# N-HANS/N-HANS

Measured on AMD Instinct MI355X. Metric: denoised audio seconds per second (16 kHz), whole job, higher is better.
Workload: dtype f16x3 (split hi+lo f16 operands, f32 accumulate); 1 GPU; 256 x 10 s 16 kHz synthetic mixture(s) per GPU, denoiser model, STFT+embed+mask+iSTFT end-to-end; clips_per_gpu=256, distinct_clips_per_gpu=256, frames_per_gpu=255488, weights=synthetic seed 7, parallelism=clip-sharded x1

## Files before the change

### include/nhans_hip.h

```cpp
#ifndef NHANS_HIP_H
#define NHANS_HIP_H

#include <stddef.h>
#include <stdint.h>

#ifdef __cplusplus
extern "C" {
#endif

#define NHANS_ABI_VERSION 5

#define NHANS_DENOISER 0
#define NHANS_SEPARATOR 1

#define NHANS_OK 0
#define NHANS_EINVAL (-1)
#define NHANS_EHIP (-2)
#define NHANS_ENOMEM (-3)
#define NHANS_ESHORT (-4)

#define NHANS_STATUS_SATURATED 1

#define NHANS_NUM_ACTIVATIONS 25

// ... 31 lines not shown

int nhans_embed(nhans_ctx* ctx, const float* ctx_logmag_dev, int n, float* emb_out_dev, void* stream);

int nhans_mask_net(nhans_ctx* ctx, const float* logmag_dev, const int64_t* frame_offsets_host,
                   int nclips, const float* emb_a_dev, const float* emb_b_dev,
                   float* logits_out_dev, float* denoised_out_dev, void* stream);

int nhans_istft(nhans_ctx* ctx, const float* logmag_dev, const float* phase_dev,
                const int64_t* frame_offsets_host, int nclips, const int64_t* out_offsets_host,
                float* wav_out_dev, void* stream);

int nhans_enhance_clips(nhans_ctx* ctx, const float* mix_wav_dev, const int64_t* mix_offsets_host,
                        int nclips, const float* ctx_a_wav_dev, const int64_t* ctx_a_offsets_host,
                        const float* ctx_b_wav_dev, const int64_t* ctx_b_offsets_host,
                        float* denoised_wav_dev, float* mixed_wav_dev, float* logmag_out_dev,
                        float* phase_out_dev, float* logits_out_dev, float* emb_out_dev, void* stream);

int nhans_debug_block_output(nhans_ctx* ctx, const float* logmag_dev, const int64_t* frame_offsets_host,
                             int nclips, const float* emb_a_dev, const float* emb_b_dev,
                             int64_t frame0, int nframes, int block, float* out_dev, void* stream);

int nhans_debug_activation(nhans_ctx* ctx, const float* logmag_dev, const int64_t* frame_offsets_host,
                           int nclips, const float* emb_a_dev, const float* emb_b_dev,
                           int64_t frame0, int nframes, int index, float* out_dev, void* stream);
int nhans_debug_tower_activation(nhans_ctx* ctx, const float* ctx_logmag_dev, int n, int index, float* out_dev,
                                 void* stream);

int nhans_take_status(nhans_ctx* ctx, int* flags_out, void* stream);

int nhans_debug_launch_probe(size_t dynamic_lds_bytes, void* stream);

int nhans_debug_mfma_ceiling(double seconds, void* stream, double* sustained_tflops, double* first_tflops,
                             int* launches);

uint32_t nhans_crc32c(uint32_t crc, const void* data_host, size_t nbytes);

typedef struct nhans_online nhans_online;

int nhans_online_open(nhans_ctx* ctx, int nstreams, const float* ctx_a_wav_dev, const int64_t* ctx_a_offsets_host,
                      const float* ctx_b_wav_dev, const int64_t* ctx_b_offsets_host, int want_mixed, void* stream,
                      nhans_online** out);

int nhans_online_open_slots(nhans_ctx* ctx, int nslots, int want_mixed, void* stream, nhans_online** out);

int nhans_online_restart(nhans_online* obj, int slot);

int nhans_online_set_context(nhans_online* obj, int slot, const float* ctx_a_wav_dev, int64_t na,
                             const float* ctx_b_wav_dev, int64_t nb, void* stream, int64_t* first_frame_out);

int nhans_online_set_embeddings(nhans_online* obj, int slot, const float* emb_a_dev, const float* emb_b_dev,
                                void* stream, int64_t* first_frame_out);


int nhans_online_push(nhans_online* obj, const float* in_dev, const int64_t* in_offsets_host, const int* end_host,
                      float* den_out_dev, float* mixed_out_dev, const int64_t* out_offsets_host,
                      int64_t* out_counts_host, void* stream);

int nhans_online_out_counts(const nhans_online* obj, const int64_t* in_counts_host, const int* end_host,
                            int64_t* out_counts_host);

int nhans_online_rewind(nhans_online* obj);

int nhans_online_set_lookahead(nhans_online* obj, int slot, int lookahead);

void nhans_online_close(nhans_online* obj);

// ... 96 lines not shown
```

### n-hans_amd/csrc/conv_epilogue.h

```cpp
#pragma once
#include "nhans_kernels.h"
#include <cstddef>

namespace nhans {

typedef float f32x16 __attribute__((ext_vector_type(16)));
typedef float f32x4 __attribute__((ext_vector_type(4)));
typedef _Float16 f16x8 __attribute__((ext_vector_type(8)));
typedef _Float16 f16x4 __attribute__((ext_vector_type(4)));

template <int I, int NM, int ND> __device__ __forceinline__ void pin_reads_between_mfmas() {
    if constexpr (I < ND) {
        __builtin_amdgcn_sched_group_barrier(0x008, (I + 1) * NM / ND - I * NM / ND, 0);
        __builtin_amdgcn_sched_group_barrier(0x100, 1, 0);
        pin_reads_between_mfmas<I + 1, NM, ND>();
    }
}

template <int I, int NM, int ND> __device__ __forceinline__ void pin_reads_front_loaded() {
    if constexpr (I < ND) {
        __builtin_amdgcn_sched_group_barrier(0x008, 1, 0);
        __builtin_amdgcn_sched_group_barrier(0x100, 1, 0);
        pin_reads_front_loaded<I + 1, NM, ND>();
    } else if constexpr (NM > ND) {
// ... 253 lines not shown
    int* const satp = CONV_KARG(sat);
    if (sat && satp) atomicOr(satp, kSatActivation);
}

template <int TM, int TN, int PREC, int NTHREADS, int BMROWS, int BNCOLS>
__device__ __forceinline__ void conv_epilogue(const ConvArgs& a, f32x16 (&acc)[TM][TN], float* smem, EpiTile tile,
                                              int row_base, int col_base, int n_tile0, int tid, int lane,
                                              long long* es = nullptr ) {
    constexpr int LDC = BNCOLS + 4;
    constexpr int C4 = BNCOLS / 4;
    constexpr int PP = NTHREADS / C4;
    constexpr int PASSES = BMROWS / PP;
    float* ct = smem;
    int4* rowinfo = reinterpret_cast<int4*>(smem + BMROWS * LDC);

#pragma unroll
    for (int i = 0; i < TM; ++i)
#pragma unroll
        for (int j = 0; j < TN; ++j)
#pragma unroll
            for (int g = 0; g < 4; ++g) {
                const f32x4 v = {acc[i][j][4 * g], acc[i][j][4 * g + 1], acc[i][j][4 * g + 2], acc[i][j][4 * g + 3]};
                *reinterpret_cast<f32x4*>(ct + (row_base + i * 32 + (lane & 31)) * LDC + col_base + j * 32 + 8 * g +
                                          4 * (lane >> 5)) = v;
            }
    if (tid < BMROWS) {
        const int mz = tile(tid, a);
        const int m = mz < 0 ? (tile.tw > 0 ? tile(0, a) : a.M - 1) : mz;
        const uint32_t b = fd_div((uint32_t)m, a.fdHoWo);
        const uint32_t rem = (uint32_t)m - b * a.fdHoWo.d;
        const uint32_t ho = fd_div(rem, a.fdWo);
        const uint32_t wo = rem - ho * a.fdWo.d;
        const int clip = a.img_clip ? a.img_clip[b] : 0;
        int ids;
        if (a.id_mode == 2 && a.id_win.t) {
            const int h = (int)ho * a.idsh;
            ids = win_row_ok(a.id_win, (int)b, h) ? win_row(a.id_win, (int)b, h) * a.idW + (int)wo * a.idsw : kNoRow;
        } else {
            ids = (int)((b * a.idH + ho * a.idsh) * a.idW + wo * a.idsw);
        }
        rowinfo[tid] = make_int4(clip * a.cb_stride, (int)rem * a.N, mz, ids);
    }
    if (kDev && es) { asm volatile("s_waitcnt lgkmcnt(0)" ::: "memory"); es[0] = (long long)__builtin_amdgcn_s_memtime(); }
    __syncthreads();
    if (kDev && es) es[1] = (long long)__builtin_amdgcn_s_memtime();

    const int c4 = tid % C4, prow = tid / C4;
    const int n = n_tile0 + c4 * 4;
    const int f_tf = a.tf ? 1 : 0;
    const bool id_split = a.id_mode == 1 && a.id_split;
    const float* __restrict__ cbp = a.cb;
    const float* __restrict__ tfp = a.tf ? a.tf : a.zero;
    const bool vec = (a.Nreal == a.N) && !a.aux && (a.out_split || (a.ldo & 3) == 0) &&
                     (a.id_mode != 1 || id_split || (a.id_ld & 3) == 0);
    constexpr int C8 = BNCOLS / 8, PP8 = NTHREADS / C8, PASSES8 = BMROWS / PP8;
    if (vec && a.epi8 && a.out_split && (a.id_mode == 0 || id_split || a.id_mode == 2)) {
        const int c8 = tid % C8, prow8 = tid / C8;
        const int n8 = n_tile0 + c8 * 8;
        const bool one_clip = rowinfo[0].x == rowinfo[BMROWS - 1].x;
        const int mode8 = (a.id_mode == 0 ? 0 : a.id_mode == 1 ? 1 : 2) * 2 + (one_clip ? 1 : 0);
        switch (mode8) {
            case 0: conv_epilogue_sweep8<PREC, 0, 0, PP8, PASSES8, LDC>(a, ct, rowinfo, prow8, c8, n8, es); break;
            case 1: conv_epilogue_sweep8<PREC, 0, 1, PP8, PASSES8, LDC>(a, ct, rowinfo, prow8, c8, n8, es); break;
            case 2: conv_epilogue_sweep8<PREC, 1, 0, PP8, PASSES8, LDC>(a, ct, rowinfo, prow8, c8, n8, es); break;
            case 3: conv_epilogue_sweep8<PREC, 1, 1, PP8, PASSES8, LDC>(a, ct, rowinfo, prow8, c8, n8, es); break;
            case 4: conv_epilogue_sweep8<PREC, 3, 0, PP8, PASSES8, LDC>(a, ct, rowinfo, prow8, c8, n8, es); break;
            default: conv_epilogue_sweep8<PREC, 3, 1, PP8, PASSES8, LDC>(a, ct, rowinfo, prow8, c8, n8, es); break;
        }
    } else if (vec) {
        const int mode = (a.id_mode == 1 ? (id_split ? 1 : 2) : a.id_mode == 2 ? 3 : 0) * 2 + (a.out_split ? 1 : 0);
        switch (mode) {
            case 0: conv_epilogue_sweep<PREC, 0, 0, PP, PASSES, LDC>(a, ct, rowinfo, prow, c4, n); break;
            case 1: conv_epilogue_sweep<PREC, 0, 1, PP, PASSES, LDC>(a, ct, rowinfo, prow, c4, n); break;
            case 2: conv_epilogue_sweep<PREC, 1, 0, PP, PASSES, LDC>(a, ct, rowinfo, prow, c4, n); break;
// ... 35 lines not shown
```

### n-hans_amd/csrc/conv_igemm_halo.hip

```cpp
#include "conv_epilogue.h"
#include <cstdlib>

namespace nhans {

namespace {
constexpr int NCW = 8;
constexpr int NPW = 4;

template <int HBM_> struct HaloShape {
    static constexpr int HBM = HBM_;
    static constexpr int HR = HBM_ == 512 ? 544 : 320;
    static constexpr int BST = HBM_ == 512 ? 3 : 4;
    static constexpr int WN = HBM_ == 512 ? 1 : 2;
    static constexpr int NAP = HR * 8 / (NPW * 64);
};

template <int N> __device__ __forceinline__ void halo_wait_vmcnt() {
    asm volatile("s_waitcnt vmcnt(%0)" ::"n"(N) : "memory");
}
}

template <int BN, int PREC, int HBM_ = 256, int DBG = 0, int ABL = 0, int PWM = 0>
__global__ void __launch_bounds__((NCW + NPW) * 64) conv_igemm_halo(const ConvArgs a) {
    using SH = HaloShape<HBM_>;
// ... 106 lines not shown
                                     (__attribute__((address_space(3))) void*)(DST), 16, 0, 0);

        int segA = 0, khA = 0, ccA = 0, supA = 0, kwA = 0;
#define NH_ISSUE_A(BUF)                                                                            \
    {                                                                                              \
        const int khoff_ = (khA * sW + (PWM ? kwA : 0)) * sC + ccA * 32;                           \
        const bool live_ = supA < nsup;                                                            \
        float* sa_ = smem + (BUF) * A_BUF + pw * 8 * 32;                                           \
        _Pragma("unroll") for (int d = 0; d < NAPW; ++d) {                                         \
            bool in_ = !(ABL & 1) && live_ && (unsigned)(hov[d] + khA) < (unsigned)sH;             \
            if constexpr (PWM) in_ = in_ && (unsigned)(wiv[d] + kwA) < (unsigned)sW;               \
            if constexpr (!(ABL & 2))                                                              \
                __builtin_amdgcn_raw_ptr_buffer_load_lds(srsrc, (__attribute__((address_space(3))) void*)(sa_ + d * 32 * 32), 16, \
                                                         in_ ? (unsigned)(poff[d] + khoff_ * 4) : kOob, 0, 0, 0); \
        }                                                                                          \
        ++supA;                                                                                    \
        if (PWM && ++kwA < KW0) {                  \
        } else if (kwA = 0, ++khA >= (segA ? KH1 : KH0)) {  \
            khA = 0;                                                                               \
            if (++ccA >= (segA ? CC1 : CC0)) {                                                     \
                ccA = 0;                                                                           \
                if (segA == 0 && nseg > 1) {                                                       \
                    segA = 1;                                                                      \
                    NH_MAP_SEGMENT(1)                                                              \
                }                                                                                  \
            }                                                                                      \
        }                                                                                          \
    }
        int tapB = 0;
        const __amdgpu_buffer_rsrc_t wr0 = __builtin_amdgcn_make_buffer_rsrc(const_cast<float*>(a.seg[0].wpk) + (size_t)nt0 * 1024, 0, 0x7FFFFFFF, 0x00020000);
        const __amdgpu_buffer_rsrc_t wr1 = __builtin_amdgcn_make_buffer_rsrc(const_cast<float*>(nseg > 1 ? a.seg[1].wpk : a.seg[0].wpk) + (size_t)nt0 * 1024, 0, 0x7FFFFFFF, 0x00020000);
        const unsigned wvo = (unsigned)ptid * 16u;
        const int bstride_b = (int)(bstride * 4);
        int wtap = -1, wseg = 0;
#define NH_ISSUE_B(ST)                                                                             \
    {                                                                                              \
        if (tapB < total && !(ABL & 4)) {                                                          \
            if (tapB == ntap0) { wseg = 1; wtap = 0; } else ++wtap;                                \
        }                                                                                          \
        ++tapB;                                                                                    \
        float* sb_ = smem + B_BASE + (ST) * B_STAGE;                                               \
        const int so_ = (ABL & 4) ? 0 : wtap * bstride_b;                                          \
        _Pragma("unroll") for (int j = 0; j < GBP; ++j)                                            \
            if constexpr (!(ABL & 8))                                                              \
                __builtin_amdgcn_raw_ptr_buffer_load_lds((wseg || (ABL & 4)) ? wr1 : wr0,          \
                    (__attribute__((address_space(3))) void*)(sb_ + (j * (NPW * 64) + pw * 64) * 4), 16, wvo, so_ + j * (NPW * 64) * 16, 0, 0); \
    }

        NH_MAP_SEGMENT(0)
        NH_ISSUE_A(0)
        NH_ISSUE_B(0)
        if constexpr (PWM) NH_ISSUE_A(1)
        NH_ISSUE_B(1)
        if constexpr (PFD == 3) NH_ISSUE_B(2)
        halo_wait_vmcnt<(PFD - 1) * GBP + (PWM ? NAPW : 0)>();
        __builtin_amdgcn_s_barrier();
        long long dbg_is = 0, dbg_vm = 0, dbg_bar = 0, dbg_t0 = 0;
        if constexpr (DBG) dbg_t0 = (long long)__builtin_amdgcn_s_memtime();
        bool prev_first = false;
        int stB = PFD;
        for (int it = 0; it < total; ++it) {
            const int KWc = segC ? 1 : KW0;
            const bool first = kwC == 0;
            long long tq0 = 0, tq1 = 0, tq2 = 0;
            if constexpr (DBG) tq0 = (long long)__builtin_amdgcn_s_memtime();
            if constexpr (PWM) {
                NH_ISSUE_A(bufC == 0 ? NABUF - 1 : bufC - 1)
            } else if (first) NH_ISSUE_A(bufC ^ 1)
            NH_ISSUE_B(stB)
            if (++stB == BST) stB = 0;
            if constexpr (DBG) tq1 = (long long)__builtin_amdgcn_s_memtime();
// ... 270 lines not shown
```

### n-hans_amd/csrc/host_ctx.hip

```cpp
#include "host_internal.h"

namespace {

thread_local std::string g_err;

constexpr uint32_t kBlobVersion = 2;
struct BlobHeader {
    char magic[8];
    uint32_t version;
    uint32_t n_entries;
    uint64_t total_bytes;
};
struct BlobEntry {
    char name[48];
    uint64_t offset;
    uint64_t nfloats;
};

std::vector<BlockGeo> tower_geometry() {
    const int kh[4] = {8, 8, 4, 4}, kw[4] = {4, 4, 4, 4}, sh[4] = {3, 3, 1, 1}, sw[4] = {2, 2, 1, 2};
    const int co[4] = {64, 128, 256, 512};
    std::vector<BlockGeo> v;
    int h = kCtxFrames, w = kBins, c = 1;
    for (int i = 0; i < 4; ++i) {
// ... 332 lines not shown
        c->lookahead = (int)value;
    }
    else if (k == "profile") c->profile = value != 0;
    else if (k == "debug_cycles_ptr") {
        if (!kDev) return fail(NHANS_EINVAL, "debug_cycles_ptr exists only in a NHANS_DEV build (make DEV=1)");
        c->dbg = reinterpret_cast<long long*>(static_cast<intptr_t>(value));
    }
    else if (k == "epilogue_wide") c->epi8 = value != 0;
    else if (k == "consumer_interleave") {
        if (value < 0 || value > 2) return fail(NHANS_EINVAL, "consumer_interleave must be 0, 1 or 2");
        c->ilv = (int)value;
    }
    else if (k == "conv_variant") {
        if (value < -1 || value > 2) return fail(NHANS_EINVAL, "conv_variant must be -1 (auto), 0, 1 or 2");
        c->conv_variant = (int)value;
    }
    else if (k == "calibrate") {
        if (value < 0 || value > 3) return fail(NHANS_EINVAL, "calibrate must be 1 (start), 0 (stop, set), 2 (stop, raise only) or 3 (stop, discard)");
        int rc = check_ctx(c); if (rc) return rc;
        if (value == 1) {
            HIP_TRY(hipDeviceSynchronize());
            HIP_TRY(hipMemset(c->amax_dev, 0, kNumAct * sizeof(unsigned)));
            c->calibrating = true;
        } else {
            if (!c->calibrating) return fail(NHANS_EINVAL, "calibrate: no bracket is open");
            if (value == 3) { c->calibrating = false; return NHANS_OK; }
            return finish_calibration(c, value == 2);
        }
    }
    else if (k == "winograd") c->wino = value != 0;
    else if (k == "winograd_f32_tensors") c->wino_f32 = (value == 2 || value == 3) ? (int)value : value != 0;
    else if (k == "split_k") c->split_k = value != 0;
    else if (k == "stream_1x1") c->stream_1x1 = value != 0;
    else if (k == "precision") {
        if (value != 0 && value != 1) return fail(NHANS_EINVAL, "precision must be 0 (f32) or 1 (f16x3)");
        if (value == 1 && !c->A("head.dense.wpk_h"))
            return fail(NHANS_EINVAL, "the folded blob carries no split-f16 weights");
        c->prec = (int)value;
    }
    else return fail(NHANS_EINVAL, "unknown option " + k);
    return NHANS_OK;
}

int nhans_set_activation_exponents(nhans_ctx* c, const int* e, int n) {
    if (!c || !e || n != kNumAct) return fail(NHANS_EINVAL, "activation exponents: need NHANS_NUM_ACTIVATIONS values");
    for (int i = 0; i < n; ++i)
        if (e[i] < -60 || e[i] > 60) return fail(NHANS_EINVAL, "activation exponent outside [-60, 60]");
    std::copy(e, e + n, c->act_exp);
    tie_exponents(c);
    return NHANS_OK;
}

int nhans_get_activation_exponents(nhans_ctx* c, int* e_out, int n) {
    if (!c || !e_out || n != kNumAct) return fail(NHANS_EINVAL, "activation exponents: need NHANS_NUM_ACTIVATIONS values");
    std::copy(c->act_exp, c->act_exp + n, e_out);
    return NHANS_OK;
}

int nhans_get_activation_amax(nhans_ctx* c, float* amax_out, int n) {
    if (!c || !amax_out || n != kNumAct) return fail(NHANS_EINVAL, "activation maxima: need NHANS_NUM_ACTIVATIONS values");
    std::copy(c->act_amax, c->act_amax + n, amax_out);
    return NHANS_OK;
}

int nhans_take_status(nhans_ctx* c, int* flags_out, void* stream) {
    int rc = check_ctx(c); if (rc) return rc;
// ... 93 lines not shown
```

### n-hans_amd/csrc/host_internal.h

```cpp
#pragma once
#include "../../include/nhans_hip.h"
#include "nhans_kernels.h"

#include <algorithm>
#include <cmath>
#include <cstdio>
#include <cstdlib>
#include <cstring>
#include <limits>
#include <map>
#include <string>
#include <vector>

using namespace nhans;

#pragma GCC visibility push(hidden)

int fail(int code, const std::string& msg);

#define HIP_TRY(expr)                                                                          \
    do {                                                                                       \
        hipError_t e_ = (expr);                                                                \
        if (e_ != hipSuccess)                                                                  \
            return fail(NHANS_EHIP, std::string(#expr) + ": " + hipGetErrorString(e_));        \
// ... 8 lines not shown
constexpr int SA(int b, int j) { return 8 + 2 * b + j; }
constexpr int kActHead = 24;

struct ProfEntry {
    int calls = 0;
    double flops = 0, bytes = 0, mfma = 0;
    std::vector<std::pair<hipEvent_t, hipEvent_t>> pending;
    double ms = 0;
};

#pragma GCC visibility pop

struct StackPlan {
    bool wino[8][3] = {};
};

struct nhans_ctx {
    int kind = 0, device = 0;
    StackPlan last_plan;
    float* blob_dev = nullptr;
    size_t blob_bytes = 0;
    std::map<std::string, const float*> arr;
    std::map<std::string, size_t> arr_n;
    std::vector<BlockGeo> tower, stack;
    int cond_cols = 0;
    std::vector<int> cond_off;
    char* ws = nullptr;
    size_t ws_bytes = 0, ws_top = 0;
    float* kscratch = nullptr;
    size_t kscratch_bytes = 0;
    static constexpr size_t kscratch_cap = (size_t)384 << 20;
    bool kscratch_failed = false;
    int stream_1x1 = 1;
    int split_k = 1;
    int* kcounter = nullptr;
    int kcounter_n = 1024;
    int64_t frames_per_chunk = 3776;
    int contexts_per_chunk = 64;
    int lookahead = kCenter;
    char* pin = nullptr;
    size_t pin_bytes = (size_t)16 << 20, pin_top = 0;
    bool profile = false;
    std::map<std::string, ProfEntry> prof;
    std::vector<hipEvent_t> event_pool;

    int prec = 0;
    int conv_variant = -1;
    int epi8 = 1;
    int ilv = 1;
    int wino = 1;
    int wino_f32 = 1;
    long long* dbg = nullptr;
    int* status_dev = nullptr;
    std::map<std::pair<int, int>, float*> rs_tab;
    int act_exp[kNumAct] = {};
    float act_amax[kNumAct] = {};
    unsigned* amax_dev = nullptr;
    bool calibrating = false;
    int cap_idx = -1;
    float* cap_out = nullptr;
    float up(int i) const { return prec ? ldexpf(1.f, act_exp[i]) : 1.f; }
    float down(int i) const { return prec ? ldexpf(1.f, -act_exp[i]) : 1.f; }
    hipEvent_t tail_ev = nullptr;
    hipStream_t last_stream = nullptr;
    bool have_tail = false;

// ... 211 lines not shown
```

### n-hans_amd/csrc/host_net.hip

```cpp
#include "host_internal.h"

namespace {

void same_pad(int n, int k, int s, int* out, int* before) {
    *out = (n + s - 1) / s;
    int total = std::max((*out - 1) * s + k - n, 0);
    *before = total / 2;
}

void fill_epilogue_defaults(nhans_ctx* c, ConvArgs& a) {
    a.zero = c->A("zero");
    a.sat = c->status_dev;
    a.img_clip = nullptr; a.tf = nullptr; a.tt = nullptr; a.ff = nullptr; a.id_mode = 0; a.id = nullptr; a.id_ld = 0;
    a.idw = nullptr; a.idH = a.idW = 0; a.idsh = a.idsw = 1; a.relu = 1; a.aux = nullptr; a.aux_ld = 0;
    a.cb_stride = 0;
    a.prec = c->prec; a.out_split = c->prec; a.id_split = 0; a.ws = nullptr;
    a.in_scale = a.id_scale = a.out_scale = 1.f;
    a.sat_limit = kSatLimitF16;
    a.variant = c->conv_variant >= 0 ? c->conv_variant : (c->prec == 1 ? 2 : 0);
    a.dbg = kDev ? c->dbg : nullptr;
    a.epi8 = c->epi8;
    a.ilv = c->ilv;
    a.wino = c->wino; a.wino_u = nullptr; a.wino_ws = nullptr;
    a.kscratch = c->kscratch; a.kscratch_bytes = c->kscratch_bytes; a.kcounter = c->kcounter; a.kcounter_n = c->kcounter_n; a.kgroup = 0;
}

ConvSeg make_seg(const float* src, const float* wpk, int H, int W, int C, int KH, int KW, int sh, int sw,
                 bool same) {
    ConvSeg g;
    g.src = src; g.wpk = wpk; g.H = H; g.W = W; g.C = C; g.KH = KH; g.KW = KW; g.sh = sh; g.sw = sw;
    int o, pb;
    if (same) { same_pad(H, KH, sh, &o, &pb); g.pt = pb; same_pad(W, KW, sw, &o, &pb); g.pl = pb; }
    else { g.pt = 0; g.pl = 0; }
    g.nchunks = KH * KW * C / 32;
    return g;
}

void set_out_geometry(ConvArgs& a, int B, int Ho, int Wo, int N, int Nreal, int ldo, float* out) {
    a.Ho = Ho; a.Wo = Wo; a.M = B * Ho * Wo; a.N = N; a.Nreal = Nreal; a.ldo = ldo; a.out = out;
    a.fdHoWo = make_fastdiv((uint32_t)(Ho * Wo));
    a.fdWo = make_fastdiv((uint32_t)Wo);
}

void run_conv(nhans_ctx* c, const ConvArgs& a0, hipStream_t s) {
    ConvArgs a = a0;
    if (kDev) {
        static const bool no_tf = [] { const char* e = getenv("NHANS_ABLATE_TF"); return e && atoi(e) != 0; }();
        if (no_tf) { a.tf = nullptr; a.tt = nullptr; a.ff = nullptr; }
    }
    if (a.kgroup < 0) {
        const size_t need = c->split_k ? conv_splitk_scratch_bytes(a) : 0;
        if (need > c->kscratch_bytes && need <= nhans_ctx::kscratch_cap && !c->kscratch_failed) {
            if (c->kscratch) { (void)hipFree(c->kscratch); c->kscratch = nullptr; c->kscratch_bytes = 0; }
            const size_t want = std::min(nhans_ctx::kscratch_cap, std::max(need, (size_t)32 << 20));
            if (hipMalloc(reinterpret_cast<void**>(&c->kscratch), want) == hipSuccess) c->kscratch_bytes = want;
            else { (void)hipGetLastError(); c->kscratch = nullptr; c->kscratch_failed = true; }
        }
        a.kscratch = c->split_k ? c->kscratch : nullptr;
        a.kscratch_bytes = c->kscratch_bytes;
    }
    Prof p(c, s, nullptr);
    const char* name = "conv_igemm";
    double mfma = 0;
    double fl = launch_conv_igemm(a, s, &name, &mfma);
    p.done(fl, 0, name, mfma);
}

bool wino_form(const ConvArgs& a) { return a.variant >= 2 && a.kgroup >= 0 && conv_wino_eligible(a); }
float sat_limit_for(const StackPlan& p, int b, int cv) { return b >= 0 && b < 8 && p.wino[b][cv] ? kSatLimitWinoInput : kSatLimitF16; }

bool stored_f32(const nhans_ctx* c, const StackPlan& p, int b, int cv) {
    if (c->prec != 1 || !c->wino_f32 || b < 0 || b > 7) return false;
    if (c->wino_f32 == 2) return b < 4 && !(b == 3 && cv == 1);
    if (c->wino_f32 == 3) return b == 1 && cv == 1;
    if (cv == 0) return p.wino[b][2] && (b == 0 || p.wino[b][1]);
    if (b == 7) return false;
    const BlockGeo& nx = c->stack[b + 1];
    return p.wino[b][2] && p.wino[b + 1][1] && nx.cin == nx.cout && p.wino[b + 1][2];
}

void tap(nhans_ctx* c, int idx, const float* buf, size_t words, int chan, hipStream_t s, bool f32_layout = false) {
    if (c->calibrating) launch_absmax(buf, words, c->prec && !f32_layout, c->up(idx), c->amax_dev + idx, s);
    if (c->cap_idx != idx) return;
    if (!c->prec) note_launch("activation tap copy", hipMemcpyAsync(c->cap_out, buf, words * 4, hipMemcpyDeviceToDevice, s));
    else if (f32_layout) launch_scale_copy(buf, words, c->up(idx), c->cap_out, s);
    else launch_unsplit(buf, (int64_t)(words / chan), chan, c->up(idx), c->cap_out, s);
    c->cap_out += words;
}

size_t stack_buf_floats(const nhans_ctx* c, int64_t wf) {
    size_t m = 0;
    for (const auto& g : c->stack) m = std::max(m, (size_t)g.hout * g.wout * g.cout);
    return m * (size_t)wf;
}

size_t transform_buf_floats(const nhans_ctx* c, int64_t wf) {
    size_t m = 0;
    for (const auto& g : c->stack)
        if (g.cin != g.cout && g.cin > 1 && g.kh == 4) m = std::max(m, (size_t)g.hout * g.wout * g.cout);
    return m * (size_t)wf;
}

float* run_stack_chunk(nhans_ctx* c, const float* logmag, const int* rb, const StackBufs& sb, int64_t g0, int n, int upto,
                       hipStream_t s) {
    StackPlan plan;
    float* result = nullptr;
    const int* clipmap = sb.f_clip + g0;
    for (int pass = 0; pass < 2; ++pass) {
    const bool go = pass == 1;
    auto dead = [&] { return go && launch_error_pending(); };
    auto conv = [&](int b, int cv, const ConvArgs& a) {
        const bool w = wino_form(a);
        if (!go) { plan.wino[b][cv] = w; return; }
        if (dead()) return;
        if (w != plan.wino[b][cv]) {
            note_refusal("stack conv whose Winograd eligibility changed between planning and launch");
            return;
        }
        run_conv(c, a, s);
    };
    const WinRows win{sb.f_t + g0, sb.f_T + g0, -kCenter, kCenter, rb ? rb + g0 : nullptr};
    const float* const lm_chunk = rb ? logmag : logmag + (size_t)g0 * kBins;
    float *x = sb.X, *a1 = sb.A, *y = sb.Y;
    for (int b = 0; b < 8 && (b < upto || !go); ++b) {
        const BlockGeo& g = c->stack[b];
        const std::string p = "m" + std::to_string(b);
        const float* cb1 = sb.cb_all + c->cond_off[2 * b];
        const float* cb2 = sb.cb_all + c->cond_off[2 * b + 1];
        if (b == 0) {
            DirectArgs d{};
            d.src = lm_chunk; d.win = win; d.w = c->A(p + ".c1.w"); d.H = g.hin; d.W = g.win; d.KH = g.kh; d.KW = g.kw;
            d.sh = 1; d.sw = 1;
            int o; same_pad(g.hin, g.kh, 1, &o, &d.pt); same_pad(g.win, g.kw, 1, &o, &d.pl);
            d.Ho = g.hout; d.Wo = g.wout; d.M = n * g.hout * g.wout; d.out = a1;
            d.cb = cb1; d.cb_stride = c->cond_cols; d.img_clip = clipmap;
            d.tf = c->A(p + ".c1.tf"); d.tt = c->A(p + ".c1.tt"); d.ff = c->A(p + ".c1.ff");
            if (!d.tt || !d.ff) d.tt = d.ff = nullptr;
            d.relu = 1; d.out_split = c->prec && !stored_f32(c, plan, 0, 0); d.sat = c->prec ? c->status_dev : nullptr;
            d.out_scale = c->down(SA(0, 0)); d.sat_limit = sat_limit_for(plan, 0, 2);
            d.fdHoWo = make_fastdiv(g.hout * g.wout); d.fdWo = make_fastdiv(g.wout);
            if (go && !dead()) {
                Prof pr(c, s, "direct_conv64");
                launch_direct_conv64(d, s);
                pr.done(2.0 * d.M * g.kh * g.kw * 64, 0);
            }
        } else {
            ConvArgs a{};
            fill_epilogue_defaults(c, a);
            a.nseg = 1;
            a.seg[0] = make_seg(x, c->WP(p + ".c1.wpk"), g.hin, g.win, g.cin, g.kh, g.kw, g.sh, g.sw, true);
            set_out_geometry(a, n, g.hout, g.wout, g.cout, g.cout, g.cout, a1);
// ... 412 lines not shown
}

int nhans_mask_net(nhans_ctx* c, const float* logmag, const int64_t* foff, int nclips, const float* ea,
                   const float* eb, float* logits, float* denoised, void* stream) {
    Call call(c, stream);
    if (call.rc) return call.rc;
    return call.finish(mask_net_body(c, logmag, foff, nclips, ea, eb, logits, denoised, stream));
}

static int debug_block_output_body(nhans_ctx* c, const float* logmag, const int64_t* foff, int nclips, const float* ea,
                             const float* eb, int64_t frame0, int nframes, int block, float* out, void* stream) {
    int rc = NHANS_OK;
    if (!logmag || !foff || !ea || !eb || !out || block < 0 || block > 8) return fail(NHANS_EINVAL, "bad argument");
    hipStream_t s = static_cast<hipStream_t>(stream);
    const int64_t total = foff[nclips];
    if (frame0 < 0 || frame0 + nframes > total) return fail(NHANS_EINVAL, "frame range outside batch");
    rc = ws_reserve(c, stack_ws_bytes(c, total, nclips, nframes)); if (rc) return rc;
    StackBufs sb;
    stack_take(c, total, nclips, nframes, &sb);
    rc = h2d(c, sb.foff_dev, foff, (nclips + 1) * sizeof(int64_t), s); if (rc) return rc;
    launch_frame_index(sb.foff_dev, nclips, total, c->lookahead, sb.f_clip, sb.f_t, sb.f_T, s);
    launch_cond(ea, eb, nclips, c->A("cond.w"), c->A("cond.base"), c->cond_cols, sb.cb_all, s);
    const float* res = run_stack_chunk(c, logmag, nullptr, sb, frame0, nframes, block + 1, s);
    size_t per;
    if (block == 8) per = (size_t)26 * 512;
    else per = (size_t)c->stack[block].hout * c->stack[block].wout * c->stack[block].cout;
    if (c->prec && block < 8 && stored_f32(c, c->last_plan, block, 1)) launch_scale_copy(res, per * nframes, c->up(SA(block, 1)), out, s);
    else if (c->prec) launch_unsplit(res, (int64_t)nframes * (int64_t)(per / (block == 8 ? 512 : c->stack[block].cout)),
                                block == 8 ? 512 : c->stack[block].cout, c->up(block == 8 ? kActHead : SA(block, 1)), out, s);
    else HIP_TRY(hipMemcpyAsync(out, res, per * nframes * 4, hipMemcpyDeviceToDevice, s));
    return NHANS_OK;
}

int nhans_debug_block_output(nhans_ctx* c, const float* logmag, const int64_t* foff, int nclips, const float* ea,
                             const float* eb, int64_t frame0, int nframes, int block, float* out, void* stream) {
    Call call(c, stream);
    if (call.rc) return call.rc;
    return call.finish(debug_block_output_body(c, logmag, foff, nclips, ea, eb, frame0, nframes, block, out, stream));
}

static int debug_activation_body(nhans_ctx* c, const float* logmag, const int64_t* foff, int nclips, const float* ea,
                                 const float* eb, int64_t frame0, int nframes, int index, float* out, void* stream) {
    int rc = NHANS_OK;
    if (!logmag || !foff || !ea || !eb || !out || nclips < 1 || nframes < 1) return fail(NHANS_EINVAL, "bad argument");
    if (index < SA(0, 0) || index >= kNumAct)
        return fail(NHANS_EINVAL, "activation index outside the stack's 8 .. " + std::to_string(kNumAct - 1) + " (tower tensors: nhans_debug_tower_activation)");
    hipStream_t s = static_cast<hipStream_t>(stream);
    const int64_t total = foff[nclips];
    if (frame0 < 0 || frame0 + nframes > total) return fail(NHANS_EINVAL, "frame range outside batch");
    const int64_t wf = std::min<int64_t>(c->frames_per_chunk, nframes);
    rc = ws_reserve(c, stack_ws_bytes(c, total, nclips, wf)); if (rc) return rc;
    StackBufs sb;
    stack_take(c, total, nclips, wf, &sb);
    rc = h2d(c, sb.foff_dev, foff, (nclips + 1) * sizeof(int64_t), s); if (rc) return rc;
    launch_frame_index(sb.foff_dev, nclips, total, c->lookahead, sb.f_clip, sb.f_t, sb.f_T, s);
    launch_cond(ea, eb, nclips, c->A("cond.w"), c->A("cond.base"), c->cond_cols, sb.cb_all, s);
    const int upto = index == kActHead ? 9 : (index - SA(0, 0)) / 2 + 1;
    c->cap_idx = index; c->cap_out = out;
    for (int64_t g0 = frame0; g0 < frame0 + nframes; g0 += wf) {
        run_stack_chunk(c, logmag, nullptr, sb, g0, (int)std::min<int64_t>(wf, frame0 + nframes - g0), upto, s);
        if (launch_error_pending()) break;
    }
    c->cap_idx = -1; c->cap_out = nullptr;
    return NHANS_OK;
}

// ... 59 lines not shown
```

### n-hans_amd/csrc/nhans_kernels.h

```cpp
#pragma once
#include <hip/hip_runtime.h>
#include <stdint.h>

#include <tuple>
#include <utility>
#include <vector>

namespace nhans {

constexpr int kWin = 400, kHop = 160, kBins = 201, kMixWin = 35, kCtxFrames = 200, kEmb = 512;
constexpr int kCenter = kMixWin / 2;
constexpr int64_t kMaxFramesPerChunk = ((int64_t)1 << 31) / ((int64_t)kMixWin * kBins * 64);

#ifdef NHANS_DEV
constexpr bool kDev = true;
int dev_ablate();
#else
constexpr bool kDev = false;
constexpr int dev_ablate() { return 0; }
#endif

void note_launch(const char* kernel, hipError_t launch_rc);
bool launch_error_pending();
void note_refusal(const char* what);
// ... 23 lines not shown
inline FastDiv make_fastdiv(uint32_t d) {
    FastDiv f;
    f.d = d;
    uint32_t l = 0;
    while ((1ull << l) < d) ++l;
    f.mul = (uint32_t)((((uint64_t)1 << 32) * (((uint64_t)1 << l) - d)) / d + 1);
    f.sh = l;
    return f;
}
__device__ __forceinline__ uint32_t fd_div(uint32_t n, const FastDiv& f) {
    return (__umulhi(f.mul, n) + n) >> f.sh;
}

struct WinRows {
    const int* t;
    const int* T;
    int row0, pad;
    const int* rb;
};
constexpr int kNoRow = -2147483647 - 1;
__device__ __forceinline__ bool win_row_ok(const WinRows& w, int b, int h) {
    return (unsigned)(w.t[b] + h - w.pad) < (unsigned)w.T[b];
}
__device__ __forceinline__ int win_row(const WinRows& w, int b, int h) {
    return (w.rb ? w.rb[b] : w.row0 + b) + h;
}

struct ConvSeg {
    const float* src;
    const float* wpk;
    int H, W, C;
    int KH, KW, sh, sw, pt, pl;
    int nchunks;
};

struct ConvArgs {
    ConvSeg seg[2];
    int nseg;
    int Ho, Wo;
    int M;
    int N;
    int Nreal;
    int ldo;
    float* out;
    const float* cb;
    int cb_stride;
    const int* img_clip;
    const float* tf;
    const float* tt;
    const float* ff;
    int id_mode;
    const float* id;
    int id_ld;
    const float* idw;
    int idH, idW, idsh, idsw;
    WinRows id_win;
    int relu;
    float* aux;
    int aux_ld;
    const float* zero;
    int prec;
    int out_split;
    int id_split;
    int in_f32;
    const float* ws;
    float in_scale, id_scale, out_scale;
    float sat_limit;
    int* sat;
    int variant;
    int epi8;
    int ilv;
    int halo64_tile512;
    long long* dbg;
// ... 153 lines not shown
```

### n-hans_amd/hip.py

```python
import ctypes
import json
import os
import sys

_HERE = os.path.dirname(os.path.abspath(__file__))
LIB_PATH = os.environ.get("NHANS_LIB") or os.path.join(_HERE, "csrc", "libnhans_hip.so")

DENOISER, SEPARATOR = 0, 1
KIND_CODE = {"denoiser": DENOISER, "separator": SEPARATOR}

_int, _i64, _dbl, _vp = ctypes.c_int, ctypes.c_int64, ctypes.c_double, ctypes.c_void_p
_size, _str = ctypes.c_size_t, ctypes.c_char_p
_ip, _i64p, _vpp = ctypes.POINTER(_int), ctypes.POINTER(_i64), ctypes.POINTER(_vp)
_fp, _dp = ctypes.POINTER(ctypes.c_float), ctypes.POINTER(_dbl)
SIGNATURES = {
    "nhans_abi_version": (_int, []),
    "nhans_last_error": (_str, []),
    "nhans_num_frames": (_i64, [_i64]),
    "nhans_create": (_int, [_int, _vp, _size, _int, _vpp]),
    "nhans_create_ex": (_int, [_int, _vp, _size, _int, _ip, _int, _vpp]),
    "nhans_destroy": (None, [_vp]),
    "nhans_set_option": (_int, [_vp, _str, _i64]),
    "nhans_set_activation_exponents": (_int, [_vp, _ip, _int]),
    "nhans_get_activation_exponents": (_int, [_vp, _ip, _int]),
    "nhans_get_activation_amax": (_int, [_vp, _fp, _int]),
    "nhans_workspace_bytes": (_size, [_vp, _i64, _int]),
    "nhans_stft_features": (_int, [_vp, _vp, _i64p, _int, _int, _vp, _vp, _vp]),
    "nhans_embed": (_int, [_vp, _vp, _int, _vp, _vp]),
    "nhans_mask_net": (_int, [_vp, _vp, _i64p, _int, _vp, _vp, _vp, _vp, _vp]),
    "nhans_istft": (_int, [_vp, _vp, _vp, _i64p, _int, _i64p, _vp, _vp]),
    "nhans_enhance_clips": (_int, [_vp, _vp, _i64p, _int, _vp, _i64p, _vp, _i64p, _vp, _vp, _vp, _vp, _vp, _vp, _vp]),
    "nhans_debug_block_output": (_int, [_vp, _vp, _i64p, _int, _vp, _vp, _i64, _int, _int, _vp, _vp]),
    "nhans_debug_activation": (_int, [_vp, _vp, _i64p, _int, _vp, _vp, _i64, _int, _int, _vp, _vp]),
    "nhans_debug_tower_activation": (_int, [_vp, _vp, _int, _int, _vp, _vp]),
    "nhans_take_status": (_int, [_vp, _ip, _vp]),
    "nhans_debug_launch_probe": (_int, [_size, _vp]),
    "nhans_debug_mfma_ceiling": (_int, [_dbl, _vp, _dp, _dp, _ip]),
    "nhans_crc32c": (ctypes.c_uint32, [ctypes.c_uint32, _vp, _size]),
    "nhans_online_open": (_int, [_vp, _int, _vp, _i64p, _vp, _i64p, _int, _vp, _vpp]),
    "nhans_online_open_slots": (_int, [_vp, _int, _int, _vp, _vpp]),
    "nhans_online_restart": (_int, [_vp, _int]),
    "nhans_online_set_context": (_int, [_vp, _int, _vp, _i64, _vp, _i64, _vp, _i64p]),
    "nhans_online_set_embeddings": (_int, [_vp, _int, _vp, _vp, _vp, _i64p]),
    "nhans_online_push": (_int, [_vp, _vp, _i64p, _ip, _vp, _vp, _i64p, _i64p, _vp]),
    "nhans_online_out_counts": (_int, [_vp, _i64p, _ip, _i64p]),
    "nhans_online_rewind": (_int, [_vp]),
    "nhans_online_set_lookahead": (_int, [_vp, _int, _int]),
    "nhans_online_close": (None, [_vp]),
    "nhans_resample_out_count": (_i64, [_i64, _int, _int]),
    "nhans_resample_emitted": (_i64, [_i64, _int, _int, _int]),
    "nhans_resample_taps": (_int, [_int, _int, _dp, _int]),
    "nhans_resample": (_int, [_vp, _vp, _int, _i64p, _int, _int, _int, _int, _vp, _i64p, _vp]),
    "nhans_peak_normalise": (_int, [_vp, _vp, _i64p, _int, _int, _vp, _vp]),
    "nhans_channel_mean": (_int, [_vp, _vp, _int, _i64, _vp, _vp]),
    "nhans_resampler_open": (_int, [_vp, _int, _int, _int, _int, _int, _vpp]),
    "nhans_resampler_set_peak": (_int, [_vp, _dbl]),
    "nhans_resampler_push": (_int, [_vp, _vp, _i64p, _ip, _vp, _i64p, _i64p, _vp]),
    "nhans_resampler_out_counts": (_int, [_vp, _i64p, _ip, _i64p]),
    "nhans_resampler_restart": (_int, [_vp, _int]),
    "nhans_resampler_close": (None, [_vp]),
    "nhans_live_emitted": (_i64, [_i64, _int, _int, _int]),
    "nhans_live_open_slots": (_int, [_vp, _int, _int, _int, _dbl, _int, _int, _dbl, _int, _vp, _vpp]),
    "nhans_live_restart": (_int, [_vp, _int]),
    "nhans_live_set_context": (_int, [_vp, _int, _vp, _i64, _vp, _i64, _vp, _i64p]),
    "nhans_live_set_embeddings": (_int, [_vp, _int, _vp, _vp, _vp, _i64p]),
    "nhans_live_set_wet": (_int, [_vp, _dbl]),
    "nhans_live_out_counts": (_int, [_vp, _i64p, _ip, _i64p]),
    "nhans_live_push": (_int, [_vp, _vp, _i64p, _ip, _vp, _i64p, _i64p, _vp]),
    "nhans_lookahead_live_emitted": (_i64, [_i64, _int, _int, _int, _int]),
    "nhans_lookahead_live_set": (_int, [_vp, _int, _int]),
# ... 92 lines not shown
```

Before: 503.8 audio-seconds/s.

## Split padded convolutions into row classes that skip zero-padding filter taps

Output rows of a same-padded convolution are grouped into classes by which filter rows land inside the input. Each class is launched as its own halo implicit-GEMM conv with a reduced KH, so MACs against top and bottom padding are no longer computed. The weight-tap walk in the halo kernel and the epilogue row mapping are offset so each sub-launch indexes full-filter weights and full-height outputs. This adds extra kernel launches per conv and smaller GEMMs that may fill tiles less well. A default threshold enables the split only when the skipped fraction is large enough.

```diff
diff --git a/include/nhans_hip.h b/include/nhans_hip.h
--- a/include/nhans_hip.h
+++ b/include/nhans_hip.h
@@ -87,6 +87,8 @@
 
 int nhans_debug_mfma_ceiling(double seconds, void* stream, double* sustained_tflops, double* first_tflops,
                              int* launches);
+
+int nhans_debug_row_classes(int H, int KH, int stride, int pt, int* out, int cap);
 
 uint32_t nhans_crc32c(uint32_t crc, const void* data_host, size_t nbytes);
 
diff --git a/n-hans_amd/csrc/conv_epilogue.h b/n-hans_amd/csrc/conv_epilogue.h
--- a/n-hans_amd/csrc/conv_epilogue.h
+++ b/n-hans_amd/csrc/conv_epilogue.h
@@ -309,14 +309,17 @@
         const uint32_t ho = fd_div(rem, a.fdWo);
         const uint32_t wo = rem - ho * a.fdWo.d;
         const int clip = a.img_clip ? a.img_clip[b] : 0;
+        const uint32_t hov = ho + (uint32_t)a.oh0;
+        const int remv = (int)(hov * a.fdWo.d + wo);
+        const int mv = mz < 0 ? mz : (int)(b * (uint32_t)a.Ho_full * a.fdWo.d) + remv;
         int ids;
         if (a.id_mode == 2 && a.id_win.t) {
-            const int h = (int)ho * a.idsh;
+            const int h = (int)hov * a.idsh;
             ids = win_row_ok(a.id_win, (int)b, h) ? win_row(a.id_win, (int)b, h) * a.idW + (int)wo * a.idsw : kNoRow;
         } else {
-            ids = (int)((b * a.idH + ho * a.idsh) * a.idW + wo * a.idsw);
-        }
-        rowinfo[tid] = make_int4(clip * a.cb_stride, (int)rem * a.N, mz, ids);
+            ids = (int)((b * a.idH + hov * a.idsh) * a.idW + wo * a.idsw);
+        }
+        rowinfo[tid] = make_int4(clip * a.cb_stride, remv * a.N, mv, ids);
     }
     if (kDev && es) { asm volatile("s_waitcnt lgkmcnt(0)" ::: "memory"); es[0] = (long long)__builtin_amdgcn_s_memtime(); }
     __syncthreads();
diff --git a/n-hans_amd/csrc/conv_igemm_halo.hip b/n-hans_amd/csrc/conv_igemm_halo.hip
--- a/n-hans_amd/csrc/conv_igemm_halo.hip
+++ b/n-hans_amd/csrc/conv_igemm_halo.hip
@@ -162,11 +162,18 @@
         const __amdgpu_buffer_rsrc_t wr1 = __builtin_amdgcn_make_buffer_rsrc(const_cast<float*>(nseg > 1 ? a.seg[1].wpk : a.seg[0].wpk) + (size_t)nt0 * 1024, 0, 0x7FFFFFFF, 0x00020000);
         const unsigned wvo = (unsigned)ptid * 16u;
         const int bstride_b = (int)(bstride * 4);
-        int wtap = -1, wseg = 0;
+        int wper = KH0 * KW0, wskip = (a.seg[0].KHfull - KH0) * KW0, wrun = 0;
+        int wtap = a.seg[0].kh0 * KW0 - 1, wseg = 0;
 #define NH_ISSUE_B(ST)                                                                             \
     {                                                                                              \
         if (tapB < total && !(ABL & 4)) {                                                          \
-            if (tapB == ntap0) { wseg = 1; wtap = 0; } else ++wtap;                                \
+            if (tapB == ntap0) {                                                                   \
+                wseg = 1; wtap = a.seg[1].kh0 * a.seg[1].KW; wrun = 1;                             \
+                wper = KH1 * a.seg[1].KW; wskip = (a.seg[1].KHfull - KH1) * a.seg[1].KW;           \
+            } else {                                                                               \
+                if (wrun == wper) { wrun = 0; wtap += wskip; }                                     \
+                ++wtap; ++wrun;                                                                    \
+            }                                                                                      \
         }                                                                                          \
         ++tapB;                                                                                    \
         float* sb_ = smem + B_BASE + (ST) * B_STAGE;                                               \
diff --git a/n-hans_amd/csrc/host_ctx.hip b/n-hans_amd/csrc/host_ctx.hip
--- a/n-hans_amd/csrc/host_ctx.hip
+++ b/n-hans_amd/csrc/host_ctx.hip
@@ -388,6 +388,10 @@
     else if (k == "winograd_f32_tensors") c->wino_f32 = (value == 2 || value == 3) ? (int)value : value != 0;
     else if (k == "split_k") c->split_k = value != 0;
     else if (k == "stream_1x1") c->stream_1x1 = value != 0;
+    else if (k == "row_split") {
+        if (value < 0 || value > 2) return fail(NHANS_EINVAL, "row_split must be 0, 1 or 2 (2: every conv that can be split, a measurement value)");
+        c->row_split = (int)value;
+    }
     else if (k == "precision") {
         if (value != 0 && value != 1) return fail(NHANS_EINVAL, "precision must be 0 (f32) or 1 (f16x3)");
         if (value == 1 && !c->A("head.dense.wpk_h"))
diff --git a/n-hans_amd/csrc/host_internal.h b/n-hans_amd/csrc/host_internal.h
--- a/n-hans_amd/csrc/host_internal.h
+++ b/n-hans_amd/csrc/host_internal.h
@@ -64,6 +64,7 @@
     static constexpr size_t kscratch_cap = (size_t)384 << 20;
     bool kscratch_failed = false;
     int stream_1x1 = 1;
+    int row_split = 1;
     int split_k = 1;
     int* kcounter = nullptr;
     int kcounter_n = 1024;
diff --git a/n-hans_amd/csrc/host_net.hip b/n-hans_amd/csrc/host_net.hip
--- a/n-hans_amd/csrc/host_net.hip
+++ b/n-hans_amd/csrc/host_net.hip
@@ -33,16 +33,18 @@
     if (same) { same_pad(H, KH, sh, &o, &pb); g.pt = pb; same_pad(W, KW, sw, &o, &pb); g.pl = pb; }
     else { g.pt = 0; g.pl = 0; }
     g.nchunks = KH * KW * C / 32;
+    g.kh0 = 0; g.KHfull = KH;
     return g;
 }
 
 void set_out_geometry(ConvArgs& a, int B, int Ho, int Wo, int N, int Nreal, int ldo, float* out) {
     a.Ho = Ho; a.Wo = Wo; a.M = B * Ho * Wo; a.N = N; a.Nreal = Nreal; a.ldo = ldo; a.out = out;
+    a.oh0 = 0; a.Ho_full = Ho;
     a.fdHoWo = make_fastdiv((uint32_t)(Ho * Wo));
     a.fdWo = make_fastdiv((uint32_t)Wo);
 }
 
-void run_conv(nhans_ctx* c, const ConvArgs& a0, hipStream_t s) {
+const char* run_conv(nhans_ctx* c, const ConvArgs& a0, hipStream_t s) {
     ConvArgs a = a0;
     if (kDev) {
         static const bool no_tf = [] { const char* e = getenv("NHANS_ABLATE_TF"); return e && atoi(e) != 0; }();
@@ -63,7 +65,72 @@
     const char* name = "conv_igemm";
     double mfma = 0;
     double fl = launch_conv_igemm(a, s, &name, &mfma);
+    if (a.Ho_full != a.Ho) {
+        double kfull = 0;
+        for (int i = 0; i < a.nseg; ++i) kfull += (double)a.seg[i].KHfull * a.seg[i].KW * a.seg[i].C;
+        fl = 2.0 * (double)a.M * kfull * (double)a.Nreal;
+    }
     p.done(fl, 0, name, mfma);
+    return name;
+}
+
+struct RowClass { int oh0, rows, kh0, kh; };
+
+int row_classes(int H, int KH, int s, int pt, RowClass* out, int cap) {
+    const int Ho = (H + s - 1) / s;
+    int n = 0;
+    for (int ho = 0; ho < Ho; ++ho) {
+        const int hi0 = ho * s - pt;
+        const int lo = std::max(0, -hi0), hi = std::min(KH, H - hi0);
+        if (hi <= lo) return 0;
+        if (n && out[n - 1].kh0 == lo && out[n - 1].kh == hi - lo) { ++out[n - 1].rows; continue; }
+        if (n == cap) return -1;
+        out[n++] = RowClass{ho, 1, lo, hi - lo};
+    }
+    return n;
+}
+
+bool row_split_pays(const ConvSeg& g, const RowClass* rc, int n) {
+    int applied = 0, rows = 0;
+    for (int i = 0; i < n; ++i) { applied += rc[i].rows * rc[i].kh; rows += rc[i].rows; }
+    return 100 * (rows * g.KH - applied) >= 7 * rows * g.KH;
+}
+
+constexpr int kMaxRowClasses = 8;
+bool halo_family(ConvArgs a) {
+    if (a.variant < 2 || a.kgroup != 0 || a.N % 128 != 0 || a.in_f32 || conv_wino_eligible(a)) return false;
+    a.halo64_tile512 = 0;
+    return conv_igemm_halo_eligible(a) || conv_igemm_halo_pw_eligible(a);
+}
+bool run_conv_row_classes(nhans_ctx* c, const ConvArgs& a, hipStream_t s) {
+    const ConvSeg& g = a.seg[0];
+    if (!c->row_split || a.prec != 1 || a.Ho_full != a.Ho || a.M % (a.Ho * a.Wo) != 0 || !halo_family(a)) return false;
+    if (a.nseg > 1 && a.seg[1].KH != 1) return false;
+    RowClass rc[kMaxRowClasses];
+    const int n = row_classes(g.H, g.KH, g.sh, g.pt, rc, kMaxRowClasses);
+    if (n < 2 || (g.H + g.sh - 1) / g.sh != a.Ho) return false;
+    if (c->row_split == 1 && !row_split_pays(g, rc, n)) return false;
+    const int B = a.M / (a.Ho * a.Wo);
+    ConvArgs q[kMaxRowClasses];
+    for (int i = 0; i < n; ++i) {
+        q[i] = a;
+        q[i].Ho = rc[i].rows; q[i].M = B * rc[i].rows * a.Wo; q[i].oh0 = rc[i].oh0; q[i].Ho_full = a.Ho;
+        q[i].fdHoWo = make_fastdiv((uint32_t)(rc[i].rows * a.Wo));
+        ConvSeg& h = q[i].seg[0];
+        h.KH = rc[i].kh; h.kh0 = rc[i].kh0; h.KHfull = g.KH; h.pt = g.pt - rc[i].kh0 - rc[i].oh0 * g.sh;
+        h.nchunks = h.KH * h.KW * h.C / 32;
+        if (a.nseg > 1) {
+            ConvSeg& t = q[i].seg[1];
+            if ((rc[i].oh0 + rc[i].rows - 1) * t.sh - t.pt >= t.H || rc[i].oh0 * t.sh - t.pt < 0) return false;
+            t.pt -= rc[i].oh0 * t.sh;
+        }
+        q[i].wino_u = nullptr; q[i].wino_ws = nullptr;
+        if (!halo_family(q[i])) return false;
+    }
+    for (int i = 0; i < n && !launch_error_pending(); ++i)
+        if (std::strncmp(run_conv(c, q[i], s), "conv_igemm_halo", 15) != 0)
+            note_refusal("row-class conv launch on a kernel that does not walk filter-row classes");
+    return true;
 }
 
 bool wino_form(const ConvArgs& a) { return a.variant >= 2 && a.kgroup >= 0 && conv_wino_eligible(a); }
@@ -117,6 +184,7 @@
             note_refusal("stack conv whose Winograd eligibility changed between planning and launch");
             return;
         }
+        if (!w && run_conv_row_classes(c, a, s)) return;
         run_conv(c, a, s);
     };
     const WinRows win{sb.f_t + g0, sb.f_T + g0, -kCenter, kCenter, rb ? rb + g0 : nullptr};
@@ -595,6 +663,15 @@
     return NHANS_OK;
 }
 
+int nhans_debug_row_classes(int H, int KH, int stride, int pt, int* out, int cap) {
+    if (H < 1 || KH < 1 || stride < 1 || pt < 0 || cap < 0 || (cap && !out)) return fail(NHANS_EINVAL, "row classes: bad argument");
+    std::vector<RowClass> rc((size_t)(H + stride - 1) / stride);
+    const int n = row_classes(H, KH, stride, pt, rc.data(), (int)rc.size());
+    if (n > cap) return fail(NHANS_EINVAL, "row classes: " + std::to_string(n) + " classes, room for " + std::to_string(cap));
+    for (int i = 0; i < n; ++i) { out[4 * i] = rc[i].oh0; out[4 * i + 1] = rc[i].rows; out[4 * i + 2] = rc[i].kh0; out[4 * i + 3] = rc[i].kh; }
+    return n;
+}
+
 int nhans_debug_block_output(nhans_ctx* c, const float* logmag, const int64_t* foff, int nclips, const float* ea,
                              const float* eb, int64_t frame0, int nframes, int block, float* out, void* stream) {
     Call call(c, stream);
diff --git a/n-hans_amd/csrc/nhans_kernels.h b/n-hans_amd/csrc/nhans_kernels.h
--- a/n-hans_amd/csrc/nhans_kernels.h
+++ b/n-hans_amd/csrc/nhans_kernels.h
@@ -79,6 +79,7 @@
     int H, W, C;
     int KH, KW, sh, sw, pt, pl;
     int nchunks;
+    int kh0, KHfull;
 };
 
 struct ConvArgs {
@@ -86,6 +87,7 @@
     int nseg;
     int Ho, Wo;
     int M;
+    int oh0, Ho_full;
     int N;
     int Nreal;
     int ldo;
diff --git a/n-hans_amd/hip.py b/n-hans_amd/hip.py
--- a/n-hans_amd/hip.py
+++ b/n-hans_amd/hip.py
@@ -36,6 +36,7 @@
     "nhans_take_status": (_int, [_vp, _ip, _vp]),
     "nhans_debug_launch_probe": (_int, [_size, _vp]),
     "nhans_debug_mfma_ceiling": (_int, [_dbl, _vp, _dp, _dp, _ip]),
+    "nhans_debug_row_classes": (_int, [_int, _int, _int, _int, _ip, _int]),
     "nhans_crc32c": (ctypes.c_uint32, [ctypes.c_uint32, _vp, _size]),
     "nhans_online_open": (_int, [_vp, _int, _vp, _i64p, _vp, _i64p, _int, _vp, _vpp]),
     "nhans_online_open_slots": (_int, [_vp, _int, _int, _vp, _vpp]),
```

Result: faster. 517.4 audio-seconds/s (median of 6 runs) (+2.7%).
